# anadodik/sdmm-mitsuba

Hardware: AMD Instinct MI355X
Metric: EM samples/sec (NxK resp) at K=128, N=2^20 (higher is better)
Workload: dtype f32; 1 GPU; responsibility E-step, synthetic 5D sample batch (configs[1]); K=128, N=1048576, global_batch=1048576, samples_per_gpu=1048576, parallelism=sample-sharded x1 (strong: N fixed), layout=SoA fp32 in, [N][K] fp32 out

## Files before the change

### include/sdmm_gpu.h

```cpp
#ifndef SDMM_GPU_H
#define SDMM_GPU_H

#include <stddef.h>
#include <stdint.h>

#ifdef __cplusplus
extern "C" {
#endif

#define SDMM_ABI_VERSION 1

enum {
    SDMM_OK = 0,
    SDMM_E_INVALID = -1,
    SDMM_E_HIP = -2,
    SDMM_E_STATE = -3,
    SDMM_E_NOMEM = -4
};

typedef struct sdmm_mix sdmm_mix;

typedef struct {
    float alpha;
    float bprior[5];
// ... 8 lines not shown
    const float* hpdf;
    const uint8_t* is_diffuse;
    int64_t n;
} sdmm_samples;

void sdmm_em_params_default(sdmm_em_params* p);

int sdmm_create(int K, const sdmm_em_params* params, int device, sdmm_mix** out);
int sdmm_create_on_stream(int K, const sdmm_em_params* params, int device, void* hip_stream, sdmm_mix** out);
int sdmm_create_many_on_stream(int K, const sdmm_em_params* params, int device, void* hip_stream, int n,
                               sdmm_mix** out);
void sdmm_destroy(sdmm_mix* m);
int sdmm_num_components(const sdmm_mix* m);
int sdmm_layout(const sdmm_mix* m, int* resp_cpl, int* resp_lps, int* stats_cpl, int* stats_lps);
const char* sdmm_kernel_name(const sdmm_mix* m, int which);
int sdmm_set_guide_capacity(sdmm_mix* m, int cap);
int sdmm_set_guide_order(sdmm_mix* m, int coherent);
int sdmm_guide_fallback_count(const sdmm_mix* m, int* count);
int sdmm_set_stream(sdmm_mix* m, void* hip_stream);
void* sdmm_get_stream(const sdmm_mix* m);
int sdmm_synchronize(sdmm_mix* m);

int sdmm_init_hemisphere(sdmm_mix* m, const float* positions, const float* normals, int n_pos,
                         float depth_prior, float min_spatial_distance, uint64_t seed);

int sdmm_init_hemisphere_batched(sdmm_mix* const* mixes, int n, const float* positions, const float* normals,
                                 float depth_prior, const float* min_spatial_distance, const uint64_t* seeds);

int sdmm_kmeanspp_select(const sdmm_samples* s, const float* const normals[3], const int64_t* seg, int n_leaves,
                         int n_pos, const float* uniforms, int device, void* hip_stream, int64_t* out_index,
// ... 322 lines not shown
```

### sdmm-mitsuba_amd/__init__.py

```python
from __future__ import annotations

import ctypes as C
import os
from pathlib import Path

import numpy as np

PKG_DIR = Path(__file__).resolve().parent
LIB_PATH = Path(os.environ.get("SDMM_LIB_PATH", PKG_DIR / "lib" / "libsdmm_amd.so"))
REPO = PKG_DIR.parent


class SDMMError(RuntimeError):
    pass


_lib = None


def build(arch: str = "gfx950", jobs: int = 4) -> Path:
    import subprocess
    subprocess.run(["make", "-s", f"-j{jobs}", "-C", str(PKG_DIR), f"ARCH={arch}"], check=True)
    return LIB_PATH

# ... 181 lines not shown
                ("out", C.c_void_p), ("out_stride", C.c_int64), ("comp", C.c_void_p)]


def _check(rc: int):
    if rc != 0:
        raise SDMMError(f"sdmm error {rc}: {lib().sdmm_last_error().decode()}")


def stats_len(K: int) -> int:
    return 2 + 21 * K


EXPORTED_SYMBOLS = [
    "sdmm_release_cached_scratch",
    "sdmm_em_params_default", "sdmm_create", "sdmm_destroy", "sdmm_num_components", "sdmm_layout",
    "sdmm_kernel_name",
    "sdmm_set_guide_capacity", "sdmm_set_guide_order", "sdmm_guide_fallback_count",
    "sdmm_set_stream", "sdmm_get_stream", "sdmm_synchronize", "sdmm_init_hemisphere",
    "sdmm_hemisphere_init_host", "sdmm_em_step", "sdmm_em_step_host", "sdmm_em_step_batched",
    "sdmm_em_step_batched_host",
    "sdmm_stats_len",
    "sdmm_estep_stats", "sdmm_mstep", "sdmm_responsibilities", "sdmm_guide_batch", "sdmm_pdf_batch",
    "sdmm_sample_discrete_cdf", "sdmm_get_params", "sdmm_set_params", "sdmm_get_state",
    "sdmm_set_state", "sdmm_last_error", "sdmm_abi_version",
    "sdmm_stree_create", "sdmm_stree_destroy", "sdmm_stree_split_to_depth", "sdmm_stree_split",
    "sdmm_stree_num_nodes", "sdmm_stree_get_nodes", "sdmm_stree_find", "sdmm_stree_route",
    "sdmm_stree_set_stream", "sdmm_stree_get_stream", "sdmm_guide_wavefront", "sdmm_pdf_wavefront",
    "sdmm_stree_bind_mixtures", "sdmm_guide_product_batch", "sdmm_pdf_product_batch",
    "sdmm_save_json", "sdmm_load_json", "sdmm_mix_save_json", "sdmm_mix_load_json", "sdmm_get_em_params",
    "sdmm_restore_params", "sdmm_stree_set_nodes",
    "sdmm_comm_unique_id", "sdmm_comm_init_rccl", "sdmm_comm_init_host", "sdmm_comm_destroy", "sdmm_comm_rank",
# ... 398 lines not shown

    def set_guide_capacity(self, cap: int):
        _check(lib().sdmm_set_guide_capacity(self.h, cap))

    def guide_fallback_count(self) -> int:
        n = C.c_int(0)
        _check(lib().sdmm_guide_fallback_count(self.h, C.byref(n)))
        return int(n.value)

    def set_guide_order(self, coherent: bool):
        _check(lib().sdmm_set_guide_order(self.h, 1 if coherent else 0))

    def layout(self) -> dict:
        v = [C.c_int() for _ in range(4)]
        _check(lib().sdmm_layout(self.h, *[C.byref(x) for x in v]))
        return {"resp": (v[0].value, v[1].value), "stats": (v[2].value, v[3].value)}

    def kernel_name(self, which: str = "resp") -> str:
        return lib().sdmm_kernel_name(self.h, 0 if which == "resp" else 1).decode()

    def optimize(self, samples: DeviceSamples, iterations: int = 1):
        _check(lib().sdmm_em_step(self.h, samples.ptr, iterations))

    em_step = optimize

    def optimize_sharded(self, comm: "Comm", shard: DeviceSamples, iterations: int = 1):
        _check(lib().sdmm_em_step_sharded(self.h, comm.h, shard.ptr, iterations))

    def estep_stats(self, samples: DeviceSamples, stats):
        assert stats.numel() >= stats_len(self.K) and stats.is_cuda
        _check(lib().sdmm_estep_stats(self.h, samples.ptr, stats.data_ptr()))
# ... 898 lines not shown
```

### sdmm-mitsuba_amd/csrc/estep_split.hip

```cpp
#include "sdmm_device.h"

namespace sdmm {

namespace {

typedef float f2 __attribute__((ext_vector_type(2)));
typedef float f4 __attribute__((ext_vector_type(4)));
typedef __bf16 bf8 __attribute__((ext_vector_type(8)));
typedef __bf16 bf2 __attribute__((ext_vector_type(2)));
typedef unsigned u4 __attribute__((ext_vector_type(4)));

template <bool B> struct Tag { static constexpr bool value = B; };

constexpr float kLog2Norm5S = -6.628740082514092f;

__device__ __forceinline__ f2 spl(float x) { return (f2)(x); }
__device__ __forceinline__ f2 pfma(f2 a, f2 b, f2 c) { return __builtin_elementwise_fma(a, b, c); }
__device__ __forceinline__ f2 pmul(f2 a, f2 b) { return a * b; }
__device__ __forceinline__ f2 padd(f2 a, f2 b) { return a + b; }

__device__ __forceinline__ unsigned pk(float lo, float hi) {
    const bf2 v = __builtin_convertvector(f2{lo, hi}, bf2);
    return __builtin_bit_cast(unsigned, v);
}
// ... 201 lines not shown
    unsigned keep;
    asm volatile(
        "s_mov_b32 %0, m0\n\t"
        "s_mov_b32 m0, %3\n\t"
        "s_nop 0\n\t"
        "global_load_lds_dword %1, off\n\t"
        "s_mov_b32 m0, %4\n\t"
        "s_nop 0\n\t"
        "global_load_lds_dword %2, off\n\t"
        "s_mov_b32 m0, %0"
        : "=&s"(keep)
        : "v"(a0), "v"(a1), "s"(lds0), "s"(lds0 + 256u)
        : "memory");
}

template <int R, int WPB, int OCC>
__global__ void __launch_bounds__(64 * WPB, OCC)
estep_resp_split_kernel(const float* __restrict__ ep, int Kp, int K, SamplesDev s, int64_t n, int64_t nwaves,
                        float* __restrict__ resp) {
    constexpr int NC = R * 8 * 64, ND = R * 4, NS = R == 8 ? 16 * 16 : 0, NF = kFeatSlots * kFeatSlotU4;
    constexpr int NTOT = WPB * NF + NC + ND + WPB * NS;
    static_assert(NTOT * 16 <= 163840, "the carved LDS block exceeds the 160 KB of a CU");
    static_assert(WPB * NF * 16 <= 65536, "LDS-DMA destinations stay below 64 KB");
    __shared__ u4 smem[NTOT];
    const int wid = __builtin_amdgcn_readfirstlane(threadIdx.x >> 6);
    u4* const ring = smem + wid * NF;
    u4* const cimg = smem + WPB * NF;
    f4* const dimg = (f4*)(cimg + NC);
    f4* const st = (f4*)(cimg + NC + ND + wid * NS);
    static_assert(WPB * NF + NC + ND + WPB * NS == NTOT && (R != 8 || NS == 256), "LDS carve: every region has storage");

    const float o_scene[3] = {kOrigin, kOrigin, kOrigin};
#ifdef SDMM_SPLIT_DIAG_NOIMAGE
    for (int idx = threadIdx.x; idx < NC + ND; idx += 64 * WPB) cimg[idx] = u4{0u, 0u, 0u, 0u};
#else
    for (int idx = threadIdx.x; idx < NC; idx += 64 * WPB)
        cimg[idx] = coef_frag(ep, Kp, idx >> 9, (idx >> 6) & 7, idx & 63, o_scene);
    for (int i = threadIdx.x; i < ND; i += 64 * WPB) {
        const float* d = ep + EP_DIPI * Kp + 4 * i;
        dimg[i] = f4{d[0], d[1], d[2], d[3]};
    }
#endif
    __syncthreads();

    const int lane = threadIdx.x & 63;
    static_assert(WPB % 4 == 0, "the deal numbers a workgroup's waves in quads");
    const int64_t wave = 4 * ((int64_t)(wid >> 2) * gridDim.x + blockIdx.x) + (wid & 3);
    const int64_t s0 = 16 * wave, step = 16 * nwaves, s1 = n;
    if (wave >= nwaves || s0 >= n) return;
    const uint64_t span = (uint64_t)(s1 - s0), whole = span - 16;
    const int jfull = span < 16          ? 0
                      : (whole >> 32) == 0 ? (int)((uint32_t)whole / (uint32_t)step) + 1
                                           : (int)(whole / (uint64_t)step) + 1;
    const int64_t tl = s0 + jfull * step;
    const int rows_last = tl < s1 ? (int)(s1 - tl) : 0;
    const int nit = jfull + (rows_last > 0 ? 1 : 0);

// ... 180 lines not shown
        S = rows_sum4(S);
        const float S2 = dif ? fmaf(1.0f - kHeuristicWeight, S, kHeuristicWeight * hp) : S;
        const float inv = __builtin_amdgcn_rcpf(S2);
        const bool fin = __builtin_isfinite(inv) && !dzero;
        gsc_p = fin ? (dif ? inv * (1.0f - kHeuristicWeight) : inv) : 0.0f;
        const bool bad = __builtin_amdgcn_ballot_w64(!__builtin_isfinite(S)) != 0;
        full_p = rows == 16 && (16 * R == K) && !bad;
        rowp = rowt;
        rows_p = rows;
        rowt += rowstep;
    }
    flush();
    wait_vm<0>();
}

#ifndef SDMM_SPLIT_R8_WPB
#define SDMM_SPLIT_R8_WPB 12
#define SDMM_SPLIT_R8_OCC 3
#endif
#define SDMM_SPLIT_CONFIGS(X) X(1, 4, 4) X(2, 4, 4) X(4, 4, 4) X(8, SDMM_SPLIT_R8_WPB, SDMM_SPLIT_R8_OCC)

static void split_cfg(int R, int , int* wpb, int* occ) {
    *wpb = 4;
    *occ = 4;
    if (R == 8) {
        *wpb = SDMM_SPLIT_R8_WPB;
        *occ = SDMM_SPLIT_R8_OCC;
    }
}

bool estep_resp_split_supported(int Kp) { return Kp % 16 == 0 && Kp / 16 <= 8 && (Kp / 16 & (Kp / 16 - 1)) == 0; }

hipError_t launch_estep_resp_split(int variant, const float* ep, int Kp, int K, const SamplesDev& s, int64_t n,
                                   int64_t resident_waves, float* resp, hipStream_t st) {
    if (!estep_resp_split_supported(Kp) || K > Kp || resident_waves <= 0) return hipErrorInvalidValue;
    const int R = Kp / 16;
    int wpb, occ;
    split_cfg(R, variant, &wpb, &occ);
    const int64_t tiles = (n + 15) / 16;
    const int64_t blocks = ((tiles < resident_waves ? tiles : resident_waves) + wpb - 1) / wpb;
    const int64_t waves = blocks * wpb;
    if (waves >= (int64_t)1 << 26) return hipErrorInvalidValue;
#define X(RR, WW, OO)                                                                                          \
    if (R == RR && wpb == WW && occ == OO) {                                                                   \
        hipLaunchKernelGGL((estep_resp_split_kernel<RR, WW, OO>), dim3((unsigned)blocks), dim3(64 * WW), 0, st, ep, \
                           Kp, K, s, n, waves, resp);                                                          \
        return hipGetLastError();                                                                              \
    }
    SDMM_SPLIT_CONFIGS(X)
#undef X
    return hipErrorInvalidValue;
}

hipError_t estep_resp_split_occupancy(int variant, int Kp, int* waves_per_cu) {
    const int R = Kp / 16;
    int wpb, occ;
    split_cfg(R, variant, &wpb, &occ);
    int blocks = 0;
#define X(RR, WW, OO)                                                                                          \
    if (R == RR && wpb == WW && occ == OO) {                                                                   \
        hipError_t e = hipOccupancyMaxActiveBlocksPerMultiprocessor(                                           \
            &blocks, reinterpret_cast<const void*>(&estep_resp_split_kernel<RR, WW, OO>), 64 * WW, 0);         \
        *waves_per_cu = blocks * WW;                                                                           \
        return e;                                                                                              \
    }
    SDMM_SPLIT_CONFIGS(X)
#undef X
    return hipErrorInvalidValue;
}

const char* estep_resp_split_name(int variant, int Kp) {
    static thread_local char buf[64];
    int wpb, occ;
    split_cfg(Kp / 16, variant, &wpb, &occ);
    snprintf(buf, sizeof buf, "estep_resp_split_kernel<%d,%d,%d>", Kp / 16, wpb, occ);
    return buf;
}

}
```

### sdmm-mitsuba_amd/csrc/sdmm_api.cpp

```cpp
#include <hip/hip_runtime.h>
#include <rccl/rccl.h>

#include <cmath>
#include <cstdlib>
#include <cstdio>
#include <cstring>
#include <new>
#include <string>
#include <vector>
#include <algorithm>
#include <atomic>
#include <future>
#include <thread>
#include <mutex>

#include "../../include/sdmm_gpu.h"
#include "sdmm_device.h"
#include "render_device.h"
#include "host_xfer.h"

#pragma clang fp contract(off)

namespace sdmm {
hipError_t launch_estep_resp(int cpl, int lps, const float* ep, int Kp, int K, const SamplesDev& s,
// ... 4 lines not shown
                              const int2* items = nullptr);
hipError_t launch_reduce_finalize_batched(const float* partials, int pstride, int Kp, int K,
                                          const LeafDesc* leaves, int n_leaves, hipStream_t st);
hipError_t launch_mstep_batched(int K, int Kp, const MixDesc* mixes, int n_mix, float norm5, hipStream_t st);
hipError_t launch_set_f64(double* p, double v, hipStream_t st);
hipError_t estep_occupancy(int cpl, int lps, int Kp, int* resp_blocks, int* stats_blocks);
hipError_t launch_estep_resp_tile(int variant, const float* ep, int Kp, int K, const SamplesDev& s, int64_t n,
                                  int64_t chunk, float* resp, hipStream_t st);
hipError_t estep_resp_tile_occupancy(int variant, int* blocks_per_cu);
const char* estep_resp_tile_name(int variant);
hipError_t launch_estep_resp_mfma(int variant, const float* ep, int Kp, int K, const SamplesDev& s, int64_t n,
                                  int64_t chunk, float* resp, hipStream_t st);
hipError_t estep_resp_mfma_occupancy(int variant, int Kp, int* blocks_per_cu);
const char* estep_resp_mfma_name(int variant, int Kp);
bool estep_resp_split_supported(int Kp);
hipError_t launch_estep_resp_split(int variant, const float* ep, int Kp, int K, const SamplesDev& s, int64_t n,
                                   int64_t resident_waves, float* resp, hipStream_t st);
hipError_t estep_resp_split_occupancy(int variant, int Kp, int* waves_per_cu);
const char* estep_resp_split_name(int variant, int Kp);
hipError_t launch_estep_stats_tile(int variant, const float* ep, int Kp, int K, const SamplesDev& s, int64_t n,
                                   int64_t chunk, int blocks, float* partials, int pstride, hipStream_t st,
                                   const LeafDesc* leaves = nullptr, const int2* items = nullptr);
hipError_t estep_stats_tile_occupancy(int variant, int Kp, int* blocks_per_cu);
hipError_t launch_reduce_partials(const float* partials, int rows, int pstride, const float* ep_for_finalize,
                                  int Kp, int K, double* stats, hipStream_t st);
hipError_t launch_set_all(int K, int Kp, const double* mean, const double* cov, const CanonDev& C,
                          float* ep, float* gp, float norm5, hipStream_t st);
hipError_t launch_pack_all(int K, int Kp, const CanonDev& C, float* ep, float* gp, float norm5,
                           hipStream_t st);
hipError_t launch_init_state(int K, const double* scal, const float* bprior, float eps, double* sc, float* bp,
                             float* bd, hipStream_t st);
hipError_t launch_hemi_gen_batched(int n, int K, const float* pos, const float* nrm, const float* dist,
                                   const uint64_t* seed, int skip, float depth_prior, void* staging, size_t per,
                                   hipStream_t st);
// ... 379 lines not shown
    mutable GuideSortScratch guide_sort{};
    mutable ProductScratch product_scratch{};
    int guide_order = 1;
    hipStream_t stream = nullptr;
    hipStream_t own_stream = nullptr;
    sdmm_em_params params{};
    float norm2 = 0, norm3 = 0, norm5 = 0;
    bool initialised = false;

    void* block = nullptr;
    struct Slab* slab = nullptr;
    CanonDev C{};
    EmStateDev S{};
    float* ep = nullptr;
    float* gp = nullptr;
    double* stats = nullptr;
    double* tmp_mean = nullptr;
    double* tmp_cov = nullptr;
    unsigned* mcount = nullptr;
    float* partials = nullptr;
    int partial_rows = 0;
    int pstride = 0;
    void* staging = nullptr;
    size_t staging_bytes = 0;
    void* batch_dev = nullptr;
    void* batch_host = nullptr;
    mutable void* it_dev = nullptr;
    mutable void* it_host = nullptr;
    mutable size_t it_cap = 0;
    size_t batch_bytes = 0;
// ... 54 lines not shown
    }
    int r = comm_pinned(c, bytes);
    if (r) return r;
    HIP_TRY(hipMemcpyAsync(c->pinned, dbuf, bytes, hipMemcpyDeviceToHost, st));
    HIP_TRY(hipStreamSynchronize(st));
    if (c->h_broadcast(c->pinned, bytes, root, c->user) != 0)
        return fail(SDMM_E_STATE, "host broadcast callback failed");
    HIP_TRY(hipMemcpyAsync(dbuf, c->pinned, bytes, hipMemcpyHostToDevice, st));
    HIP_TRY(hipStreamSynchronize(st));
    return SDMM_OK;
}

}

namespace {

int choose_layout(int K, int& cpl, int& lps) {
    if (K <= 16) { lps = 8; cpl = 2; }
    else if (K <= 32) { lps = 16; cpl = 2; }
    else if (K <= 64) { lps = 32; cpl = 2; }
    else if (K <= 128) { lps = 64; cpl = 2; }
    else if (K <= 256) { lps = 64; cpl = 4; }
    else if (K <= 512) { lps = 64; cpl = 8; }
    else return -1;
    return 0;
}

struct Split {
    int64_t chunk;
    int blocks;
// ... 250 lines not shown
    if (K > 64 && K <= 128) { m->rcpl = 4; m->rlps = 32; }
    {
        const char* ev = std::getenv("SDMM_RESP_KERNEL");
        const bool legacy = ev && std::strcmp(ev, "legacy") == 0;
        const bool mfma = ev && std::strcmp(ev, "mfma") == 0;
        const bool tile = ev && std::strcmp(ev, "tile") == 0;
        const bool split = ev && std::strcmp(ev, "split") == 0;
        if (K > 64 && K <= 128 && !legacy && !mfma) {
            m->rtile = 1;
            m->rcpl = 2;
            m->rlps = 64;
            if (!tile && estep_resp_split_supported(m->Kp)) m->rtile = 3;
        }
        if (mfma) m->rtile = 2;
        if (split && estep_resp_split_supported(m->Kp)) m->rtile = 3;
        if (K > 64 && K <= 128) m->stile = 1;
        if (K > 128 && K <= 512) m->stile = 2;
    }
    static thread_local OccCache occ[8];
    OccCache& oc = occ[(K * 7 + device) & 7];
    const int kern = ((m->rtile * 16 + m->rvariant) * 16 + m->stile) * 16 + m->svariant;
    if (oc.K == K * 64 + device && oc.kern == kern) {
        m->resp_blocks = oc.resp;
        m->stats_blocks = oc.stats;
    } else {
        int unused = 0;
        if (estep_occupancy(m->rcpl, m->rlps, m->Kp, &m->resp_blocks, &unused) != hipSuccess ||
            estep_occupancy(m->cpl, m->lps, m->Kp, &unused, &m->stats_blocks) != hipSuccess)
            return cleanup(fail(SDMM_E_HIP, "E-step occupancy query failed"));
        if (m->rtile == 2 && estep_resp_mfma_occupancy(m->rvariant, m->Kp, &m->resp_blocks) != hipSuccess)
            return cleanup(fail(SDMM_E_HIP, "E-step occupancy query failed"));
        if (m->rtile == 3) {
            int wpc = 0;
            if (estep_resp_split_occupancy(m->rvariant, m->Kp, &wpc) != hipSuccess)
                return cleanup(fail(SDMM_E_HIP, "E-step occupancy query failed"));
            m->resp_blocks = wpc;
        }
        if (m->rtile == 1 && estep_resp_tile_occupancy(m->rvariant, &m->resp_blocks) != hipSuccess)
            return cleanup(fail(SDMM_E_HIP, "E-step occupancy query failed"));
        if (m->stile && estep_stats_tile_occupancy(m->svariant, m->Kp, &m->stats_blocks) != hipSuccess)
            return cleanup(fail(SDMM_E_HIP, "E-step occupancy query failed"));
        oc.K = K * 64 + device;
        oc.kern = kern;
        oc.resp = m->resp_blocks;
        oc.stats = m->stats_blocks;
    }
    if (on_stream) {
        m->stream = ordered;
    } else {
// ... 12 lines not shown
    if (hipMemsetAsync(m->block, 0, total, m->stream) != hipSuccess)
        return cleanup(fail(SDMM_E_HIP, "hipMemsetAsync failed"));
    layout_block(m, (char*)m->block);
    const size_t Kc = (size_t)K;
    double* sc = m->S.scalars;
    float* bp = m->S.bPriors;
    float* bd = m->S.bDepth;
    double scal[SC_COUNT];
    constructor_scalars(m, scal);
    (void)Kc;
    const float eps = (float)m->params.epsilon;
    if (launch_init_state(K, scal, m->params.bprior, eps, sc, bp, bd, m->stream) != hipSuccess)
        return cleanup(fail(SDMM_E_HIP, "state init kernel launch failed"));
    if (launch_pack_all(K, m->Kp, m->C, m->ep, m->gp, m->norm5, m->stream) != hipSuccess)
        return cleanup(fail(SDMM_E_HIP, "pack kernel launch failed"));
    if (!on_stream && hipStreamSynchronize(m->stream) != hipSuccess)
        return cleanup(fail(SDMM_E_HIP, "hipStreamSynchronize failed"));
    *out = m;
    return SDMM_OK;
}

int create_many(int K, const sdmm_em_params* params, int device, hipStream_t st, int n, sdmm_mix** out) {
    if (n < 0 || (n > 0 && !out)) return fail(SDMM_E_INVALID, "invalid argument");
    for (int i = 0; i < n; ++i) out[i] = nullptr;
    if (n == 0) return SDMM_OK;
    if (hipSetDevice(device) != hipSuccess) return fail(SDMM_E_HIP, "hipSetDevice failed");
    Slab* slab = new (std::nothrow) Slab();
    if (!slab) return fail(SDMM_E_NOMEM, "out of host memory");
    slab->st = st;
    sdmm_mix probe;
// ... 15 lines not shown
        fail_at = inject ? std::atoi(inject) : -1;
        if (fail_at >= 0) std::fprintf(stderr, "sdmm: debug fault injection at create_many member %d\n", fail_at);
    }
    for (int i = 0; i < n && !r; ++i) {
        if (i == fail_at) { r = fail(SDMM_E_HIP, "create_many: injected failure"); break; }
        r = create_impl(K, params, device, st, true, &out[i], (char*)slab->p + stride * (size_t)i);
        if (!r) { out[i]->slab = slab; ++slab->refs; }
    }
    hipError_t e = r ? hipSuccess : hipMemsetAsync(slab->p, 0, stride * (size_t)n, st);
    if (!r && e == hipSuccess) {
        sdmm_mix* m0 = out[0];
        double scal[SC_COUNT];
        constructor_scalars(m0, scal);
        e = launch_init_pack_many(n, K, m0->Kp, scal, m0->params.bprior, (float)m0->params.epsilon, m0->S.scalars,
                                  m0->S.bPriors, m0->S.bDepth, m0->C, m0->ep, m0->gp, m0->norm5, stride, st);
    }
    if (r || e != hipSuccess) {
        ++slab->refs;
        for (int i = 0; i < n; ++i) { sdmm_destroy(out[i]); out[i] = nullptr; }
        if (--slab->refs == 0) { (void)hipFreeAsync(slab->p, st); delete slab; }
        return r ? r : fail(SDMM_E_HIP, std::string("create_many: ") + hipGetErrorString(e));
    }
    return SDMM_OK;
}

}

extern "C" {

void sdmm_destroy(sdmm_mix* m) { sdmm_detail::destroy_impl(m, true); }
// ... 2 lines not shown

void sdmm_detail::destroy_impl(sdmm_mix* m, bool sync) {
    if (!m) return;
    (void)hipSetDevice(m->device);
    if (sync && m->own_stream) (void)hipStreamSynchronize(m->own_stream);
    if (sync && m->stream && m->stream != m->own_stream) (void)hipStreamSynchronize(m->stream);
    if (m->slab) {
        if (--m->slab->refs == 0) {
            (void)hipFreeAsync(m->slab->p, m->stream);
            delete m->slab;
        }
    } else if (m->block) {
        (void)hipFree(m->block);
    }
    if (m->partials) (void)hipFree(m->partials);
    if (m->guide_fb) (void)hipFree(m->guide_fb);
    if (m->product_scratch.base) (void)hipFree(m->product_scratch.base);
    if (m->staging) (void)hipFree(m->staging);
    if (m->batch_dev) (void)hipFree(m->batch_dev);
    if (m->batch_host) (void)hipHostFree(m->batch_host);
    if (m->it_dev) (void)hipFree(m->it_dev);
    if (m->it_host) (void)hipHostFree(m->it_host);
    if (m->shard_stats) (void)hipFree(m->shard_stats);
    if (m->batch_copied) (void)hipEventDestroy(m->batch_copied);
    if (m->batch_done) (void)hipEventDestroy(m->batch_done);
    if (m->own_stream) (void)hipStreamDestroy(m->own_stream);
    delete m;
}

void sdmm_detail::destroy_many(sdmm_mix* const* ms, int n) {
// ... 23 lines not shown
namespace {

int copy_prefix_many(const sdmm_mix* const* src, sdmm_mix* const* dst, int n, hipStream_t st) {
    for (int i = 0; i < n; ++i)
        if (src[i]->stream != st) HIP_TRY(hipStreamSynchronize(src[i]->stream));
    const size_t bytes = (size_t)((char*)src[0]->stats - (char*)src[0]->C.weights);
    const size_t tb = sizeof(void*) * 2 * (size_t)n;
    char* pin = nullptr;
    HIP_TRY(bounce_buf(tb, &pin));
    void** ptrs = (void**)pin;
    for (int i = 0; i < n; ++i) {
        dst[i]->params = src[i]->params;
        dst[i]->guide_cap = src[i]->guide_cap;
        dst[i]->guide_order = src[i]->guide_order;
        dst[i]->initialised = src[i]->initialised;
        ptrs[(size_t)i] = src[i]->C.weights;
        ptrs[(size_t)n + i] = dst[i]->C.weights;
    }
    StreamScratch* ss = nullptr;
    std::unique_lock<std::mutex> hold = stream_scratch(src[0]->device, st, &ss);
    hipError_t e = scratch_reserve(*ss, tb);
    void* dtab = ss->p;
    if (e == hipSuccess) e = hipMemcpyAsync(dtab, ptrs, tb, hipMemcpyHostToDevice, st);
    if (e == hipSuccess) e = launch_copy_many(n, dtab, (void**)dtab + n, bytes, st);
    {
        const hipError_t es = hipStreamSynchronize(st);
        if (e == hipSuccess) e = es;
    }
    if (e != hipSuccess) return fail(SDMM_E_HIP, std::string("mixture copy: ") + hipGetErrorString(e));
    return SDMM_OK;
// ... 71 lines not shown
    HIP_TRY(hipSetDevice(m->device));
    HIP_TRY(hipMemcpyAsync(count, m->guide_fb, sizeof(int), hipMemcpyDeviceToHost, m->stream));
    HIP_TRY(hipStreamSynchronize(m->stream));
    return SDMM_OK;
}

int sdmm_layout(const sdmm_mix* m, int* resp_cpl, int* resp_lps, int* stats_cpl, int* stats_lps) {
    if (!m) return fail(SDMM_E_INVALID, "null handle");
    if (resp_cpl) *resp_cpl = m->rcpl;
    if (resp_lps) *resp_lps = m->rlps;
    if (stats_cpl) *stats_cpl = m->cpl;
    if (stats_lps) *stats_lps = m->lps;
    return SDMM_OK;
}

const char* sdmm_kernel_name(const sdmm_mix* m, int which) {
    if (!m) return "";
    static thread_local char buf[64];
    if (which == 0) {
        if (m->rtile == 3) {
            std::snprintf(buf, sizeof buf, "%s", estep_resp_split_name(m->rvariant, m->Kp));
            return buf;
        } else if (m->rtile == 2) {
            std::snprintf(buf, sizeof buf, "%s", estep_resp_mfma_name(m->rvariant, m->Kp));
            return buf;
        } else if (m->rtile) {
            std::snprintf(buf, sizeof buf, "%s", estep_resp_tile_name(m->rvariant));
            return buf;
        }
        std::snprintf(buf, sizeof buf, "estep_resp_kernel<%d,%d>", m->rcpl, m->rlps);
        return buf;
    }
    if (m->stile == 2)
        std::snprintf(buf, sizeof buf, "estep_stats_tile_kernel<%d,2,true>", m->Kp / 128);
    else if (m->stile)
        std::snprintf(buf, sizeof buf, "estep_stats_tile_kernel<4,%d>", m->svariant == 1 ? 3 : 2);
// ... 29 lines not shown
    return SDMM_OK;
}

static int upload_and_set(sdmm_mix* m, const float* weights, const float* means, const float* covs) {
    const size_t K = (size_t)m->K;
    char* pin = nullptr;
    HIP_TRY(bounce_buf(8 * 31 * K + 4 * K, &pin));
    double* md = (double*)pin;
    double* cd = md + 6 * K;
    for (size_t i = 0; i < 6 * K; ++i) md[i] = (double)means[i];
    for (size_t i = 0; i < 25 * K; ++i) cd[i] = (double)covs[i];
    std::memcpy(cd + 25 * K, weights, 4 * K);
    HIP_TRY(hipMemcpyAsync(m->tmp_mean, md, 8 * 6 * K, hipMemcpyHostToDevice, m->stream));
    HIP_TRY(hipMemcpyAsync(m->tmp_cov, cd, 8 * 25 * K, hipMemcpyHostToDevice, m->stream));
    HIP_TRY(hipMemcpyAsync(m->C.weights, cd + 25 * K, 4 * K, hipMemcpyHostToDevice, m->stream));
    HIP_TRY(launch_set_all(m->K, m->Kp, m->tmp_mean, m->tmp_cov, m->C, m->ep, m->gp, m->norm5, m->stream));
    HIP_TRY(hipStreamSynchronize(m->stream));
    m->initialised = true;
    return SDMM_OK;
}

static int init_hemisphere_batched_impl(sdmm_mix* const* mixes, int n, const float* positions,
                                        const float* normals, float depth_prior, const float* min_spatial_distance,
                                        const uint64_t* seeds, int skip);

int sdmm_init_hemisphere(sdmm_mix* m, const float* positions, const float* normals, int n_pos,
                         float depth_prior, float min_spatial_distance, uint64_t seed) {
    if (!m) return fail(SDMM_E_INVALID, "handle is NULL");
    HIP_TRY(hipSetDevice(m->device));
    if (n_pos * 8 != m->K) return fail(SDMM_E_INVALID, "K must equal 8 * n_pos");
// ... 85 lines not shown
        for (int t = 1; t < nt; ++t) {
            const int a = (int)((int64_t)n * t / nt), b = (int)((int64_t)n * (t + 1) / nt);
            try {
                th.emplace_back(init_range, a, b);
            } catch (...) {
                init_range(a, b);
            }
        }
        init_range(0, (int)((int64_t)n / nt));
        for (auto& x : th) x.join();
    }
    InitDescHost* tab = (InitDescHost*)(pin + stage_bytes - up_off);
    for (int i = 0; i < n; ++i) {
        sdmm_mix* m = mixes[i];
        tab[i] = InitDescHost{m->C, m->ep, m->gp, m->S.bPriors, m->S.bDepth, m->tmp_mean, m->tmp_cov};
    }
    const size_t in_off = stage_bytes + tab_bytes;
    const size_t dist_off = in_off + 2 * pn_bytes;
    const size_t seed_off = (dist_off + sizeof(float) * (size_t)n + 7) / 8 * 8;
    if (!host_gen) {
        std::memcpy(pin + in_off - up_off, positions, pn_bytes);
        std::memcpy(pin + in_off - up_off + pn_bytes, normals, pn_bytes);
        std::memcpy(pin + dist_off - up_off, min_spatial_distance, sizeof(float) * (size_t)n);
        std::memcpy(pin + seed_off - up_off, seeds, sizeof(uint64_t) * (size_t)n);
    }
    const size_t total = stage_bytes + tab_bytes + in_bytes;
    hipError_t e0 = r ? hipSuccess : scratch_reserve(*ss, total);
    char* d = ss->p;
    if (!r && e0 == hipSuccess) e0 = hipMemcpyAsync(d + up_off, pin, total - up_off, hipMemcpyHostToDevice, st);
    if (!r && e0 == hipSuccess && !host_gen)
// ... 61 lines not shown
    if (!m->initialised) return fail(SDMM_E_STATE, "mixture not initialised");
    HIP_TRY(hipSetDevice(m->device));
    int r = check_samples(s);
    if (r) return r;
    if (s->n == 0) {
        HIP_TRY(hipMemsetAsync(stats, 0, 8 * sdmm_stats_len(m->K), m->stream));
        return SDMM_OK;
    }
    return run_estep_stats(m, s, stats);
}

int sdmm_mstep(sdmm_mix* m, const double* stats, int64_t n_total) {
    if (!m || !stats) return fail(SDMM_E_INVALID, "invalid argument");
    if (!m->initialised) return fail(SDMM_E_STATE, "mixture not initialised");
    HIP_TRY(hipSetDevice(m->device));
    HIP_TRY(launch_mstep(m->K, m->Kp, stats, n_total, m->C, m->S, m->ep, m->gp, m->norm5, m->tmp_mean,
                         m->mcount, m->stream));
    return SDMM_OK;
}

int sdmm_comm_unique_id(void* id) {
    if (!id) return fail(SDMM_E_INVALID, "id is NULL");
    ncclUniqueId u;
    const ncclResult_t r = ncclGetUniqueId(&u);
    if (r != ncclSuccess) return nccl_fail(r, "ncclGetUniqueId");
    std::memcpy(id, &u, sizeof(u));
    return SDMM_OK;
}

int sdmm_comm_init_rccl(const void* id, int nranks, int rank, int device, sdmm_comm** out) {
// ... 54 lines not shown
    if (!m || !c) return fail(SDMM_E_INVALID, "invalid argument");
    if (!m->initialised) return fail(SDMM_E_STATE, "mixture not initialised");
    if (c->device != m->device) return fail(SDMM_E_INVALID, "communicator on another device");
    int r = check_samples(shard);
    if (r) return r;
    HIP_TRY(hipSetDevice(m->device));
    const size_t len = sdmm_stats_len(m->K);
    for (int it = 0; it < iterations; ++it) {
        if (shard->n == 0) {
            HIP_TRY(hipMemsetAsync(m->stats, 0, 8 * len, m->stream));
        } else if ((r = run_estep_stats(m, shard, m->stats))) {
            return r;
        }
        HIP_TRY(launch_set_f64(m->stats + len, (double)shard->n, m->stream));
        if ((r = comm_allreduce(c, m->stats, len + 1, m->stream))) return r;
        HIP_TRY(launch_mstep(m->K, m->Kp, m->stats, -1, m->C, m->S, m->ep, m->gp, m->norm5, m->tmp_mean,
                             m->mcount, m->stream));
    }
    return SDMM_OK;
}

int sdmm_mix_broadcast(sdmm_mix* const* mixes, int n_mix, const int32_t* owner, sdmm_comm* c) {
    if (n_mix < 0 || !c || (n_mix > 0 && (!mixes || !owner))) return fail(SDMM_E_INVALID, "invalid argument");
    if (n_mix == 0) return SDMM_OK;
    for (int i = 0; i < n_mix; ++i) {
        if (!mixes[i]) return fail(SDMM_E_INVALID, "NULL handle in mixes");
        if (owner[i] < 0 || owner[i] >= c->nranks) return fail(SDMM_E_INVALID, "owner rank out of range");
        if (mixes[i]->device != c->device) return fail(SDMM_E_INVALID, "mixture on another device");
        if (mixes[i]->K != mixes[0]->K) return fail(SDMM_E_INVALID, "mixtures must share K");
    }
    HIP_TRY(hipSetDevice(c->device));
    const hipStream_t st = mixes[0]->stream;
    for (int i = 1; i < n_mix; ++i)
        if (mixes[i]->stream != st) HIP_TRY(hipStreamSynchronize(mixes[i]->stream));
    const size_t bytes = (size_t)((char*)mixes[0]->stats - (char*)mixes[0]->C.weights);
    if (c->nccl) {
        ncclResult_t g = ncclGroupStart();
        if (g != ncclSuccess) return nccl_fail(g, "ncclGroupStart");
        for (int i = 0; i < n_mix; ++i) {
            const int r = comm_broadcast(c, mixes[i]->C.weights, bytes, owner[i], st);
            if (r) { (void)ncclGroupEnd(); return r; }
        }
        g = ncclGroupEnd();
        if (g != ncclSuccess) return nccl_fail(g, "ncclGroupEnd");
    } else {
        for (int i = 0; i < n_mix; ++i) {
            const int r = comm_broadcast(c, mixes[i]->C.weights, bytes, owner[i], st);
            if (r) return r;
        }
    }
// ... 1 lines not shown
    HIP_TRY(hipStreamSynchronize(st));
    return SDMM_OK;
}

int sdmm_clone(const sdmm_mix* src, sdmm_mix** out) {
    if (!src || !out) return fail(SDMM_E_INVALID, "invalid argument");
    *out = nullptr;
    sdmm_mix* m = nullptr;
    int r = sdmm_create_on_stream(src->K, &src->params, src->device, (void*)src->stream, &m);
    if (r) return r;
    m->guide_cap = src->guide_cap;
    m->guide_order = src->guide_order;
    const size_t bytes = (size_t)((char*)src->stats - (char*)src->C.weights);
    hipError_t e = hipSetDevice(src->device);
    if (e == hipSuccess) e = hipMemcpyAsync(m->C.weights, src->C.weights, bytes, hipMemcpyDeviceToDevice, m->stream);
    if (e != hipSuccess) {
        sdmm_destroy(m);
        return fail(SDMM_E_HIP, std::string("sdmm_clone: ") + hipGetErrorString(e));
    }
    m->initialised = src->initialised;
    *out = m;
    return SDMM_OK;
}

int sdmm_em_step(sdmm_mix* m, const sdmm_samples* s, int iterations) {
    if (!m) return fail(SDMM_E_INVALID, "handle is NULL");
    if (!m->initialised) return fail(SDMM_E_STATE, "mixture not initialised");
    HIP_TRY(hipSetDevice(m->device));
    int r = check_samples(s);
    if (r) return r;
    if (s->n == 0) return SDMM_OK;
    for (int it = 0; it < iterations; ++it) {
        r = run_estep_stats(m, s, m->stats);
        if (r) return r;
        HIP_TRY(launch_mstep(m->K, m->Kp, m->stats, s->n, m->C, m->S, m->ep, m->gp, m->norm5, m->tmp_mean,
                             m->mcount, m->stream));
    }
    return SDMM_OK;
}

}

namespace {

int check_batch(sdmm_mix* const* mixes, int n_mix, const sdmm_samples* s, const int64_t* s0, const int64_t* cnt) {
    std::vector<const sdmm_mix*> seen;
    seen.reserve((size_t)n_mix);
    const sdmm_mix* m0 = mixes[0];
    for (int i = 0; i < n_mix; ++i) {
// ... 133 lines not shown
    char* hb = (char*)m0->batch_host;
    char* db = (char*)m0->batch_dev;
    LeafDesc* leaves = (LeafDesc*)hb;
    MixDesc* mixd = (MixDesc*)(hb + off_mix);
    int2* items = (int2*)(hb + off_items);
    double* counts = (double*)(hb + off_cnt);
    const double* dcounts = (const double*)(db + off_cnt);
    int row = 0;
    for (int i = 0; i < n_mix; ++i) {
        sdmm_mix* m = mixes[i];
        const int64_t n = cnt[i] > 0 ? cnt[i] : 0;
        double* lstats = comm ? sh + len * (size_t)i : m->stats;
        leaves[i] = LeafDesc{m->ep, lstats, s0[i], n, plans[(size_t)i].chunk, row, plans[(size_t)i].blocks};
        mixd[i] = MixDesc{m->C, m->S, m->ep, m->gp, lstats, m->tmp_mean, m->tmp_cov, cnt[i] < 0 ? 0 : n,
                          (comm && cnt[i] >= 0) ? sh + len * (size_t)n_mix + i : nullptr};
        counts[i] = (double)n;
        for (int b = 0; b < plans[(size_t)i].blocks; ++b) items[row + b] = int2{i, b};
        row += plans[(size_t)i].blocks;
    }
    HIP_TRY(hipMemcpyAsync(db, hb, need, hipMemcpyHostToDevice, st));
    HIP_TRY(hipEventRecord(m0->batch_copied, st));
    const LeafDesc* dleaves = (const LeafDesc*)db;
    const MixDesc* dmix = (const MixDesc*)(db + off_mix);
    const int2* ditems = (const int2*)(db + off_items);
    const SamplesDev d = to_dev(s);
    if (rows > 0)
        HIP_TRY(launch_stats_kernel(m0, d, 0, StatsPlan{0, 0}, (int)rows, m0->partials, st, dleaves, ditems));
    HIP_TRY(launch_reduce_finalize_batched(m0->partials, m0->pstride, m0->Kp, m0->K, dleaves, n_mix, st));
    if (comm) {
        HIP_TRY(hipMemcpyAsync(sh + len * (size_t)n_mix, dcounts, sizeof(double) * (size_t)n_mix,
// ... 101 lines not shown
    const hipError_t e = hipStreamSynchronize(m->stream);
    if (r) return r;
    if (e != hipSuccess) return fail(SDMM_E_HIP, std::string("sdmm_em_step_host: ") + hipGetErrorString(e));
    return SDMM_OK;
}

int sdmm_responsibilities(sdmm_mix* m, const sdmm_samples* s, float* resp) {
    if (!m || !resp) return fail(SDMM_E_INVALID, "invalid argument");
    if (!m->initialised) return fail(SDMM_E_STATE, "mixture not initialised");
    HIP_TRY(hipSetDevice(m->device));
    int r = check_samples(s);
    if (r) return r;
    if (s->n == 0) return SDMM_OK;
    if (m->rtile == 3) {
        const int64_t resident = (int64_t)m->cus * (m->resp_blocks > 0 ? m->resp_blocks : 1);
        HIP_TRY(launch_estep_resp_split(m->rvariant, m->ep, m->Kp, m->K, to_dev(s), s->n, resident, resp, m->stream));
        return SDMM_OK;
    }
    if (m->rtile == 2) {
        const int64_t resident = (int64_t)m->cus * 4 * (m->resp_blocks > 0 ? m->resp_blocks : 1);
        int64_t chunk = (s->n + 3 * resident - 1) / (3 * resident);
        chunk = ((chunk + 15) / 16) * 16;
        if (chunk < 64) chunk = 64;
        HIP_TRY(launch_estep_resp_mfma(m->rvariant, m->ep, m->Kp, m->K, to_dev(s), s->n, chunk, resp, m->stream));
        return SDMM_OK;
    }
    if (m->rtile) {
        const int64_t resident = (int64_t)m->cus * 4 * (m->resp_blocks > 0 ? m->resp_blocks : 1);
        int64_t chunk = (s->n + 3 * resident - 1) / (3 * resident);
        chunk = ((chunk + 63) / 64) * 64;
        if (chunk < 64) chunk = 64;
// ... 121 lines not shown
    const int r = xfer(items, (int)(sizeof(items) / sizeof(items[0])), false, m->stream);
    if (r) return r;
    return SDMM_OK;
}

int sdmm_set_state(sdmm_mix* m, const double* scalars, const double* T, const double* sgW, const double* sgM,
                   const double* sgC, const float* bpriors, const float* bdepth) {
    if (!m) return fail(SDMM_E_INVALID, "handle is NULL");
    HIP_TRY(hipSetDevice(m->device));
    const size_t K = (size_t)m->K;
    const XferItem items[] = {
        {(void*)scalars, m->S.scalars, 8 * SC_COUNT}, {(void*)T, m->S.T, 8 * K}, {(void*)sgW, m->S.sgW, 8 * K},
        {(void*)sgM, m->S.sgM, 40 * K}, {(void*)sgC, m->S.sgC, 200 * K}, {(void*)bpriors, m->S.bPriors, 100 * K},
        {(void*)bdepth, m->S.bDepth, 36 * K},
    };
    const int r = xfer(items, (int)(sizeof(items) / sizeof(items[0])), true, m->stream);
    if (r) return r;
    return SDMM_OK;
}

int sdmm_get_em_params(const sdmm_mix* m, sdmm_em_params* p) {
    if (!m || !p) return fail(SDMM_E_INVALID, "invalid argument");
    *p = m->params;
    return SDMM_OK;
}

int sdmm_restore_params(sdmm_mix* m, const sdmm_params_out* in) {
    if (!m || !in) return fail(SDMM_E_INVALID, "invalid argument");
    const size_t K = (size_t)m->K;
    hipStream_t st = m->stream;
    const XferItem items[] = {
        {in->weights, m->C.weights, 4 * K}, {in->cdf, m->C.cdf, 4 * K}, {in->mean, m->C.mean, 24 * K},
        {in->cov, m->C.cov, 100 * K}, {in->to, m->C.to, 36 * K}, {in->cholL, m->C.cholL, 100 * K},
        {in->cholLInv, m->C.cholLInv, 100 * K}, {in->detInv, m->C.detInv, 4 * K},
        {in->muPremult, m->C.muPremult, 24 * K}, {in->condCov, m->C.condCov, 16 * K},
        {in->margL, m->C.margL, 36 * K}, {in->margDetInv, m->C.margDetInv, 4 * K},
        {in->condL, m->C.condL, 16 * K}, {in->condLInv, m->C.condLInv, 16 * K},
        {in->condDetInv, m->C.condDetInv, 4 * K}, {(void*)in->valid, m->C.valid, 4 * K},
    };
    for (const XferItem& it : items)
        if (!it.host) return fail(SDMM_E_INVALID, "sdmm_restore_params: every array is required");
    HIP_TRY(hipSetDevice(m->device));
    const int r = xfer(items, (int)(sizeof(items) / sizeof(items[0])), true, st);
    if (r) return r;
    HIP_TRY(launch_pack_all(m->K, m->Kp, m->C, m->ep, m->gp, m->norm5, st));
    HIP_TRY(hipStreamSynchronize(st));
    m->initialised = true;
    return SDMM_OK;
}

}

struct STNodeHost {
    float mn[3], mx[3];
    int axis = 0;
    int child[2] = {-1, -1};
};
// ... 1272 lines not shown
```

Baseline: 6.988 billion samples/s.

## Cache precomputed responsibility coefficient image across E-step calls

Every block of the split responsibility kernel used to rebuild the coefficient/LDS image from the packed parameters. The image is now built once into global memory by a separate kernel and reused until an epoch counter shows the parameters changed. Each block then only copies the ready image into LDS, which cuts the per-block prologue work. The cost is an extra buffer, epoch bookkeeping at every parameter write site, and a risk of stale images if any write path is missed.

```diff
diff --git a/include/sdmm_gpu.h b/include/sdmm_gpu.h
--- a/include/sdmm_gpu.h
+++ b/include/sdmm_gpu.h
@@ -46,6 +46,7 @@
 int sdmm_num_components(const sdmm_mix* m);
 int sdmm_layout(const sdmm_mix* m, int* resp_cpl, int* resp_lps, int* stats_cpl, int* stats_lps);
 const char* sdmm_kernel_name(const sdmm_mix* m, int which);
+int sdmm_resp_image_builds(const sdmm_mix* m, int64_t* count);
 int sdmm_set_guide_capacity(sdmm_mix* m, int cap);
 int sdmm_set_guide_order(sdmm_mix* m, int coherent);
 int sdmm_guide_fallback_count(const sdmm_mix* m, int* count);
diff --git a/sdmm-mitsuba_amd/__init__.py b/sdmm-mitsuba_amd/__init__.py
--- a/sdmm-mitsuba_amd/__init__.py
+++ b/sdmm-mitsuba_amd/__init__.py
@@ -219,7 +219,7 @@
 EXPORTED_SYMBOLS = [
     "sdmm_release_cached_scratch",
     "sdmm_em_params_default", "sdmm_create", "sdmm_destroy", "sdmm_num_components", "sdmm_layout",
-    "sdmm_kernel_name",
+    "sdmm_kernel_name", "sdmm_resp_image_builds",
     "sdmm_set_guide_capacity", "sdmm_set_guide_order", "sdmm_guide_fallback_count",
     "sdmm_set_stream", "sdmm_get_stream", "sdmm_synchronize", "sdmm_init_hemisphere",
     "sdmm_hemisphere_init_host", "sdmm_em_step", "sdmm_em_step_host", "sdmm_em_step_batched",
@@ -648,7 +648,14 @@
     def layout(self) -> dict:
         v = [C.c_int() for _ in range(4)]
         _check(lib().sdmm_layout(self.h, *[C.byref(x) for x in v]))
-        return {"resp": (v[0].value, v[1].value), "stats": (v[2].value, v[3].value)}
+        out = {"resp": (v[0].value, v[1].value), "stats": (v[2].value, v[3].value)}
+        fn = getattr(lib(), "sdmm_resp_image_builds", None)
+        if fn is not None:
+            fn.argtypes = [C.c_void_p, C.POINTER(C.c_int64)]
+            cnt = C.c_int64()
+            _check(fn(self.h, C.byref(cnt)))
+            out["resp_image_builds"] = cnt.value
+        return out
 
     def kernel_name(self, which: str = "resp") -> str:
         return lib().sdmm_kernel_name(self.h, 0 if which == "resp" else 1).decode()
diff --git a/sdmm-mitsuba_amd/csrc/estep_split.hip b/sdmm-mitsuba_amd/csrc/estep_split.hip
--- a/sdmm-mitsuba_amd/csrc/estep_split.hip
+++ b/sdmm-mitsuba_amd/csrc/estep_split.hip
@@ -239,10 +239,24 @@
         : "memory");
 }
 
-template <int R, int WPB, int OCC>
-__global__ void __launch_bounds__(64 * WPB, OCC)
-estep_resp_split_kernel(const float* __restrict__ ep, int Kp, int K, SamplesDev s, int64_t n, int64_t nwaves,
-                        float* __restrict__ resp) {
+__device__ __forceinline__ u4 image_entry(const float* __restrict__ ep, int Kp, int idx, int nc) {
+    const float o_scene[3] = {kOrigin, kOrigin, kOrigin};
+    if (idx < nc) return coef_frag(ep, Kp, idx >> 9, (idx >> 6) & 7, idx & 63, o_scene);
+    const float* d = ep + EP_DIPI * Kp + 4 * (idx - nc);
+    return __builtin_bit_cast(u4, f4{d[0], d[1], d[2], d[3]});
+}
+
+__global__ void __launch_bounds__(256) estep_resp_image_kernel(const float* __restrict__ ep, int Kp,
+                                                               u4* __restrict__ img) {
+    const int R = Kp / 16, nc = R * 8 * 64, nd = R * 4;
+    const int idx = blockIdx.x * 256 + threadIdx.x;
+    if (idx < nc + nd) img[idx] = image_entry(ep, Kp, idx, nc);
+}
+
+template <int R, int WPB, bool INLINE>
+__device__ __forceinline__ void resp_split_body(const float* __restrict__ ep, const u4* __restrict__ img, int Kp, int K,
+                                                const SamplesDev& s, int64_t n, int64_t nwaves,
+                                                float* __restrict__ resp) {
     constexpr int NC = R * 8 * 64, ND = R * 4, NS = R == 8 ? 16 * 16 : 0, NF = kFeatSlots * kFeatSlotU4;
     constexpr int NTOT = WPB * NF + NC + ND + WPB * NS;
     static_assert(NTOT * 16 <= 163840, "the carved LDS block exceeds the 160 KB of a CU");
@@ -255,17 +269,22 @@
     f4* const st = (f4*)(cimg + NC + ND + wid * NS);
     static_assert(WPB * NF + NC + ND + WPB * NS == NTOT && (R != 8 || NS == 256), "LDS carve: every region has storage");
 
-    const float o_scene[3] = {kOrigin, kOrigin, kOrigin};
-#ifdef SDMM_SPLIT_DIAG_NOIMAGE
-    for (int idx = threadIdx.x; idx < NC + ND; idx += 64 * WPB) cimg[idx] = u4{0u, 0u, 0u, 0u};
-#else
-    for (int idx = threadIdx.x; idx < NC; idx += 64 * WPB)
-        cimg[idx] = coef_frag(ep, Kp, idx >> 9, (idx >> 6) & 7, idx & 63, o_scene);
-    for (int i = threadIdx.x; i < ND; i += 64 * WPB) {
-        const float* d = ep + EP_DIPI * Kp + 4 * i;
-        dimg[i] = f4{d[0], d[1], d[2], d[3]};
-    }
-#endif
+    if constexpr (INLINE) {
+        for (int idx = threadIdx.x; idx < NC + ND; idx += 64 * WPB) cimg[idx] = image_entry(ep, Kp, idx, NC);
+    } else {
+        constexpr int T = 64 * WPB, TRIPS = (NC + ND + T - 1) / T;
+        u4 v[TRIPS];
+#pragma unroll
+        for (int i = 0; i < TRIPS; ++i) {
+            const int idx = (int)threadIdx.x + i * T;
+            v[i] = img[idx < NC + ND ? idx : NC + ND - 1];
+        }
+#pragma unroll
+        for (int i = 0; i < TRIPS; ++i) {
+            const int idx = (int)threadIdx.x + i * T;
+            if (idx < NC + ND) cimg[idx] = v[i];
+        }
+    }
     __syncthreads();
 
     const int lane = threadIdx.x & 63;
@@ -476,6 +495,20 @@
     wait_vm<0>();
 }
 
+template <int R, int WPB, int OCC>
+__global__ void __launch_bounds__(64 * WPB, OCC)
+estep_resp_split_kernel(const float* __restrict__ ep, const u4* __restrict__ img, int Kp, int K, SamplesDev s,
+                        int64_t n, int64_t nwaves, float* __restrict__ resp) {
+    resp_split_body<R, WPB, false>(ep, img, Kp, K, s, n, nwaves, resp);
+}
+
+template <int R, int WPB, int OCC>
+__global__ void __launch_bounds__(64 * WPB, OCC)
+estep_resp_split_inline_kernel(const float* __restrict__ ep, int Kp, int K, SamplesDev s, int64_t n, int64_t nwaves,
+                               float* __restrict__ resp) {
+    resp_split_body<R, WPB, true>(ep, nullptr, Kp, K, s, n, nwaves, resp);
+}
+
 #ifndef SDMM_SPLIT_R8_WPB
 #define SDMM_SPLIT_R8_WPB 12
 #define SDMM_SPLIT_R8_OCC 3
@@ -493,8 +526,18 @@
 
 bool estep_resp_split_supported(int Kp) { return Kp % 16 == 0 && Kp / 16 <= 8 && (Kp / 16 & (Kp / 16 - 1)) == 0; }
 
-hipError_t launch_estep_resp_split(int variant, const float* ep, int Kp, int K, const SamplesDev& s, int64_t n,
-                                   int64_t resident_waves, float* resp, hipStream_t st) {
+size_t estep_resp_image_bytes(int Kp) { return (size_t)(Kp / 16) * (8 * 64 + 4) * 16; }
+
+hipError_t launch_estep_resp_image(const float* ep, int Kp, void* img, hipStream_t st) {
+    if (!estep_resp_split_supported(Kp) || !img) return hipErrorInvalidValue;
+    const int entries = (Kp / 16) * (8 * 64 + 4);
+    hipLaunchKernelGGL(estep_resp_image_kernel, dim3((unsigned)((entries + 255) / 256)), dim3(256), 0, st, ep, Kp,
+                       (u4*)img);
+    return hipGetLastError();
+}
+
+hipError_t launch_estep_resp_split(int variant, const float* ep, const void* img, int Kp, int K, const SamplesDev& s,
+                                   int64_t n, int64_t resident_waves, float* resp, hipStream_t st) {
     if (!estep_resp_split_supported(Kp) || K > Kp || resident_waves <= 0) return hipErrorInvalidValue;
     const int R = Kp / 16;
     int wpb, occ;
@@ -505,8 +548,12 @@
     if (waves >= (int64_t)1 << 26) return hipErrorInvalidValue;
 #define X(RR, WW, OO)                                                                                          \
     if (R == RR && wpb == WW && occ == OO) {                                                                   \
-        hipLaunchKernelGGL((estep_resp_split_kernel<RR, WW, OO>), dim3((unsigned)blocks), dim3(64 * WW), 0, st, ep, \
-                           Kp, K, s, n, waves, resp);                                                          \
+        if (img)                                                                                               \
+            hipLaunchKernelGGL((estep_resp_split_kernel<RR, WW, OO>), dim3((unsigned)blocks), dim3(64 * WW), 0, st, \
+                               ep, (const u4*)img, Kp, K, s, n, waves, resp);                                  \
+        else                                                                                                   \
+            hipLaunchKernelGGL((estep_resp_split_inline_kernel<RR, WW, OO>), dim3((unsigned)blocks), dim3(64 * WW), \
+                               0, st, ep, Kp, K, s, n, waves, resp);                                           \
         return hipGetLastError();                                                                              \
     }
     SDMM_SPLIT_CONFIGS(X)
@@ -514,7 +561,7 @@
     return hipErrorInvalidValue;
 }
 
-hipError_t estep_resp_split_occupancy(int variant, int Kp, int* waves_per_cu) {
+hipError_t estep_resp_split_occupancy(int variant, int Kp, bool inline_image, int* waves_per_cu) {
     const int R = Kp / 16;
     int wpb, occ;
     split_cfg(R, variant, &wpb, &occ);
@@ -522,7 +569,10 @@
 #define X(RR, WW, OO)                                                                                          \
     if (R == RR && wpb == WW && occ == OO) {                                                                   \
         hipError_t e = hipOccupancyMaxActiveBlocksPerMultiprocessor(                                           \
-            &blocks, reinterpret_cast<const void*>(&estep_resp_split_kernel<RR, WW, OO>), 64 * WW, 0);         \
+            &blocks,                                                                                           \
+            inline_image ? reinterpret_cast<const void*>(&estep_resp_split_inline_kernel<RR, WW, OO>)          \
+                         : reinterpret_cast<const void*>(&estep_resp_split_kernel<RR, WW, OO>),                \
+            64 * WW, 0);                                                                                       \
         *waves_per_cu = blocks * WW;                                                                           \
         return e;                                                                                              \
     }
@@ -531,11 +581,11 @@
     return hipErrorInvalidValue;
 }
 
-const char* estep_resp_split_name(int variant, int Kp) {
+const char* estep_resp_split_name(int variant, int Kp, bool inline_image) {
     static thread_local char buf[64];
     int wpb, occ;
     split_cfg(Kp / 16, variant, &wpb, &occ);
-    snprintf(buf, sizeof buf, "estep_resp_split_kernel<%d,%d,%d>", Kp / 16, wpb, occ);
+    snprintf(buf, sizeof buf, "estep_resp_split%s_kernel<%d,%d,%d>", inline_image ? "_inline" : "", Kp / 16, wpb, occ);
     return buf;
 }
 
diff --git a/sdmm-mitsuba_amd/csrc/sdmm_api.cpp b/sdmm-mitsuba_amd/csrc/sdmm_api.cpp
--- a/sdmm-mitsuba_amd/csrc/sdmm_api.cpp
+++ b/sdmm-mitsuba_amd/csrc/sdmm_api.cpp
@@ -42,10 +42,12 @@
 hipError_t estep_resp_mfma_occupancy(int variant, int Kp, int* blocks_per_cu);
 const char* estep_resp_mfma_name(int variant, int Kp);
 bool estep_resp_split_supported(int Kp);
-hipError_t launch_estep_resp_split(int variant, const float* ep, int Kp, int K, const SamplesDev& s, int64_t n,
-                                   int64_t resident_waves, float* resp, hipStream_t st);
-hipError_t estep_resp_split_occupancy(int variant, int Kp, int* waves_per_cu);
-const char* estep_resp_split_name(int variant, int Kp);
+size_t estep_resp_image_bytes(int Kp);
+hipError_t launch_estep_resp_image(const float* ep, int Kp, void* img, hipStream_t st);
+hipError_t launch_estep_resp_split(int variant, const float* ep, const void* img, int Kp, int K, const SamplesDev& s,
+                                   int64_t n, int64_t resident_waves, float* resp, hipStream_t st);
+hipError_t estep_resp_split_occupancy(int variant, int Kp, bool inline_image, int* waves_per_cu);
+const char* estep_resp_split_name(int variant, int Kp, bool inline_image);
 hipError_t launch_estep_stats_tile(int variant, const float* ep, int Kp, int K, const SamplesDev& s, int64_t n,
                                    int64_t chunk, int blocks, float* partials, int pstride, hipStream_t st,
                                    const LeafDesc* leaves = nullptr, const int2* items = nullptr);
@@ -455,6 +457,11 @@
     EmStateDev S{};
     float* ep = nullptr;
     float* gp = nullptr;
+    bool rimg_inline = false;
+    void* rimg = nullptr;
+    uint64_t ep_epoch = 1;
+    uint64_t rimg_epoch = 0;
+    int64_t rimg_builds = 0;
     double* stats = nullptr;
     double* tmp_mean = nullptr;
     double* tmp_cov = nullptr;
@@ -539,6 +546,8 @@
 }
 
 namespace {
+
+inline void ep_written(sdmm_mix* m) { ++m->ep_epoch; }
 
 int choose_layout(int K, int& cpl, int& lps) {
     if (K <= 16) { lps = 8; cpl = 2; }
@@ -819,12 +828,14 @@
         }
         if (mfma) m->rtile = 2;
         if (split && estep_resp_split_supported(m->Kp)) m->rtile = 3;
+        const char* iv = std::getenv("SDMM_RESP_IMAGE");
+        m->rimg_inline = iv && std::strcmp(iv, "inline") == 0;
         if (K > 64 && K <= 128) m->stile = 1;
         if (K > 128 && K <= 512) m->stile = 2;
     }
     static thread_local OccCache occ[8];
     OccCache& oc = occ[(K * 7 + device) & 7];
-    const int kern = ((m->rtile * 16 + m->rvariant) * 16 + m->stile) * 16 + m->svariant;
+    const int kern = (((m->rtile * 16 + m->rvariant) * 16 + m->stile) * 16 + m->svariant) * 2 + (m->rimg_inline ? 1 : 0);
     if (oc.K == K * 64 + device && oc.kern == kern) {
         m->resp_blocks = oc.resp;
         m->stats_blocks = oc.stats;
@@ -837,7 +848,7 @@
             return cleanup(fail(SDMM_E_HIP, "E-step occupancy query failed"));
         if (m->rtile == 3) {
             int wpc = 0;
-            if (estep_resp_split_occupancy(m->rvariant, m->Kp, &wpc) != hipSuccess)
+            if (estep_resp_split_occupancy(m->rvariant, m->Kp, m->rimg_inline, &wpc) != hipSuccess)
                 return cleanup(fail(SDMM_E_HIP, "E-step occupancy query failed"));
             m->resp_blocks = wpc;
         }
@@ -880,6 +891,7 @@
         return cleanup(fail(SDMM_E_HIP, "state init kernel launch failed"));
     if (launch_pack_all(K, m->Kp, m->C, m->ep, m->gp, m->norm5, m->stream) != hipSuccess)
         return cleanup(fail(SDMM_E_HIP, "pack kernel launch failed"));
+    ep_written(m);
     if (!on_stream && hipStreamSynchronize(m->stream) != hipSuccess)
         return cleanup(fail(SDMM_E_HIP, "hipStreamSynchronize failed"));
     *out = m;
@@ -925,6 +937,7 @@
         constructor_scalars(m0, scal);
         e = launch_init_pack_many(n, K, m0->Kp, scal, m0->params.bprior, (float)m0->params.epsilon, m0->S.scalars,
                                   m0->S.bPriors, m0->S.bDepth, m0->C, m0->ep, m0->gp, m0->norm5, stride, st);
+        for (int i = 0; i < n; ++i) ep_written(out[i]);
     }
     if (r || e != hipSuccess) {
         ++slab->refs;
@@ -957,6 +970,7 @@
         (void)hipFree(m->block);
     }
     if (m->partials) (void)hipFree(m->partials);
+    if (m->rimg) (void)hipFree(m->rimg);
     if (m->guide_fb) (void)hipFree(m->guide_fb);
     if (m->product_scratch.base) (void)hipFree(m->product_scratch.base);
     if (m->staging) (void)hipFree(m->staging);
@@ -1010,6 +1024,7 @@
         dst[i]->guide_cap = src[i]->guide_cap;
         dst[i]->guide_order = src[i]->guide_order;
         dst[i]->initialised = src[i]->initialised;
+        ep_written(dst[i]);
         ptrs[(size_t)i] = src[i]->C.weights;
         ptrs[(size_t)n + i] = dst[i]->C.weights;
     }
@@ -1111,12 +1126,18 @@
     return SDMM_OK;
 }
 
+int sdmm_resp_image_builds(const sdmm_mix* m, int64_t* count) {
+    if (!m || !count) return fail(SDMM_E_INVALID, "invalid argument");
+    *count = m->rimg_builds;
+    return SDMM_OK;
+}
+
 const char* sdmm_kernel_name(const sdmm_mix* m, int which) {
     if (!m) return "";
     static thread_local char buf[64];
     if (which == 0) {
         if (m->rtile == 3) {
-            std::snprintf(buf, sizeof buf, "%s", estep_resp_split_name(m->rvariant, m->Kp));
+            std::snprintf(buf, sizeof buf, "%s", estep_resp_split_name(m->rvariant, m->Kp, m->rimg_inline));
             return buf;
         } else if (m->rtile == 2) {
             std::snprintf(buf, sizeof buf, "%s", estep_resp_mfma_name(m->rvariant, m->Kp));
@@ -1176,6 +1197,7 @@
     HIP_TRY(hipMemcpyAsync(m->tmp_mean, md, 8 * 6 * K, hipMemcpyHostToDevice, m->stream));
     HIP_TRY(hipMemcpyAsync(m->tmp_cov, cd, 8 * 25 * K, hipMemcpyHostToDevice, m->stream));
     HIP_TRY(hipMemcpyAsync(m->C.weights, cd + 25 * K, 4 * K, hipMemcpyHostToDevice, m->stream));
+    ep_written(m);
     HIP_TRY(launch_set_all(m->K, m->Kp, m->tmp_mean, m->tmp_cov, m->C, m->ep, m->gp, m->norm5, m->stream));
     HIP_TRY(hipStreamSynchronize(m->stream));
     m->initialised = true;
@@ -1291,6 +1313,7 @@
     for (int i = 0; i < n; ++i) {
         sdmm_mix* m = mixes[i];
         tab[i] = InitDescHost{m->C, m->ep, m->gp, m->S.bPriors, m->S.bDepth, m->tmp_mean, m->tmp_cov};
+        ep_written(m);
     }
     const size_t in_off = stage_bytes + tab_bytes;
     const size_t dist_off = in_off + 2 * pn_bytes;
@@ -1382,6 +1405,7 @@
     if (!m || !stats) return fail(SDMM_E_INVALID, "invalid argument");
     if (!m->initialised) return fail(SDMM_E_STATE, "mixture not initialised");
     HIP_TRY(hipSetDevice(m->device));
+    ep_written(m);
     HIP_TRY(launch_mstep(m->K, m->Kp, stats, n_total, m->C, m->S, m->ep, m->gp, m->norm5, m->tmp_mean,
                          m->mcount, m->stream));
     return SDMM_OK;
@@ -1466,6 +1490,7 @@
         }
         HIP_TRY(launch_set_f64(m->stats + len, (double)shard->n, m->stream));
         if ((r = comm_allreduce(c, m->stats, len + 1, m->stream))) return r;
+        ep_written(m);
         HIP_TRY(launch_mstep(m->K, m->Kp, m->stats, -1, m->C, m->S, m->ep, m->gp, m->norm5, m->tmp_mean,
                              m->mcount, m->stream));
     }
@@ -1486,6 +1511,7 @@
     for (int i = 1; i < n_mix; ++i)
         if (mixes[i]->stream != st) HIP_TRY(hipStreamSynchronize(mixes[i]->stream));
     const size_t bytes = (size_t)((char*)mixes[0]->stats - (char*)mixes[0]->C.weights);
+    for (int i = 0; i < n_mix; ++i) ep_written(mixes[i]);
     if (c->nccl) {
         ncclResult_t g = ncclGroupStart();
         if (g != ncclSuccess) return nccl_fail(g, "ncclGroupStart");
@@ -1517,6 +1543,7 @@
     const size_t bytes = (size_t)((char*)src->stats - (char*)src->C.weights);
     hipError_t e = hipSetDevice(src->device);
     if (e == hipSuccess) e = hipMemcpyAsync(m->C.weights, src->C.weights, bytes, hipMemcpyDeviceToDevice, m->stream);
+    ep_written(m);
     if (e != hipSuccess) {
         sdmm_destroy(m);
         return fail(SDMM_E_HIP, std::string("sdmm_clone: ") + hipGetErrorString(e));
@@ -1536,6 +1563,7 @@
     for (int it = 0; it < iterations; ++it) {
         r = run_estep_stats(m, s, m->stats);
         if (r) return r;
+        ep_written(m);
         HIP_TRY(launch_mstep(m->K, m->Kp, m->stats, s->n, m->C, m->S, m->ep, m->gp, m->norm5, m->tmp_mean,
                              m->mcount, m->stream));
     }
@@ -1699,6 +1727,7 @@
         leaves[i] = LeafDesc{m->ep, lstats, s0[i], n, plans[(size_t)i].chunk, row, plans[(size_t)i].blocks};
         mixd[i] = MixDesc{m->C, m->S, m->ep, m->gp, lstats, m->tmp_mean, m->tmp_cov, cnt[i] < 0 ? 0 : n,
                           (comm && cnt[i] >= 0) ? sh + len * (size_t)n_mix + i : nullptr};
+        ep_written(m);
         counts[i] = (double)n;
         for (int b = 0; b < plans[(size_t)i].blocks; ++b) items[row + b] = int2{i, b};
         row += plans[(size_t)i].blocks;
@@ -1830,7 +1859,14 @@
     if (s->n == 0) return SDMM_OK;
     if (m->rtile == 3) {
         const int64_t resident = (int64_t)m->cus * (m->resp_blocks > 0 ? m->resp_blocks : 1);
-        HIP_TRY(launch_estep_resp_split(m->rvariant, m->ep, m->Kp, m->K, to_dev(s), s->n, resident, resp, m->stream));
+        if (!m->rimg_inline && m->rimg_epoch != m->ep_epoch) {
+            if (!m->rimg) HIP_TRY(hipMalloc(&m->rimg, estep_resp_image_bytes(m->Kp)));
+            HIP_TRY(launch_estep_resp_image(m->ep, m->Kp, m->rimg, m->stream));
+            m->rimg_epoch = m->ep_epoch;
+            ++m->rimg_builds;
+        }
+        HIP_TRY(launch_estep_resp_split(m->rvariant, m->ep, m->rimg_inline ? nullptr : m->rimg, m->Kp, m->K, to_dev(s),
+                                        s->n, resident, resp, m->stream));
         return SDMM_OK;
     }
     if (m->rtile == 2) {
@@ -1982,6 +2018,7 @@
         {(void*)sgM, m->S.sgM, 40 * K}, {(void*)sgC, m->S.sgC, 200 * K}, {(void*)bpriors, m->S.bPriors, 100 * K},
         {(void*)bdepth, m->S.bDepth, 36 * K},
     };
+    ep_written(m);
     const int r = xfer(items, (int)(sizeof(items) / sizeof(items[0])), true, m->stream);
     if (r) return r;
     return SDMM_OK;
@@ -2009,6 +2046,7 @@
     for (const XferItem& it : items)
         if (!it.host) return fail(SDMM_E_INVALID, "sdmm_restore_params: every array is required");
     HIP_TRY(hipSetDevice(m->device));
+    ep_written(m);
     const int r = xfer(items, (int)(sizeof(items) / sizeof(items[0])), true, st);
     if (r) return r;
     HIP_TRY(launch_pack_all(m->K, m->Kp, m->C, m->ep, m->gp, m->norm5, st));
```

After: 7.104 billion samples/s (median of 6 runs). 1.02x the previous value.
